# Jiawei-Yang/Denoising-ViT

Measured on AMD Instinct MI355X. Metric: stage-1 images denoised/sec (DINOv2-B/14, 518px, 1k Adam steps), higher is better.
Workload: dtype bf16

## Files before the change

denoising-vit_amd/csrc/dvt_fit_fused.hip:

```cpp
#include "dvt_common.h"
#include "dvt_grid_dev.h"
#include "dvt_loss_row.h"

typedef short bf16x8 __attribute__((ext_vector_type(8)));
typedef float f32x4 __attribute__((ext_vector_type(4)));

int g_fit_rows32 = 1;
int g_fit_xcd_affinity = 1;
int g_fit_small_wg = 0;

namespace {

constexpr int FR0 = 16;
constexpr int FW8 = 8;
constexpr int FE = 128;

template <bool F32>
struct Op {
  static constexpr int ES = F32 ? 4 : 2;
  static constexpr int KS = F32 ? 16 : 32;
};
typedef unsigned u32x4f __attribute__((ext_vector_type(4)));

template <bool F32>
__host__ __device__ constexpr int apitch(int K) { return K * Op<F32>::ES + 16; }

struct FusedArgs {
  DvtGridTable T;
  DvtShadowLayout S;
  DvtTLayout TL;
  int n, lattice;
  int xcd_group;
  float grad_scale;
  long long off_grid, off_b1, off_b2, off_G, off_bh1, off_bh2, off_bh3;
  DvtFusedFit f[DVT_FIT_BATCH_MAX];
};

__device__ __forceinline__ uint16_t bf16_of(float v) { return (uint16_t)(dvt_pack_bf16x2(v, 0.f) & 0xffffu); }

template <int NC, int FR, int FW, bool F32>
__device__ __forceinline__ void store_T(const char* img, void* __restrict__ dstTv, int B, int b0, int tid) {
  constexpr int RPP = F32 ? 4 : 8;
  for (int item = tid; item < NC * (FR / RPP); item += 64 * FW) {
    const int grp = item / NC, col = item - grp * NC;
    const int brow = b0 + grp * RPP;
    const char* src = img + grp * RPP * apitch<F32>(NC) + col * Op<F32>::ES;
    if constexpr (F32) {
      const int sg = brow >> 4, g = (brow >> 2) & 3;
      float4 v;
      v.x = *reinterpret_cast<const float*>(src);
      v.y = *reinterpret_cast<const float*>(src + apitch<F32>(NC));
      v.z = *reinterpret_cast<const float*>(src + 2 * apitch<F32>(NC));
      v.w = *reinterpret_cast<const float*>(src + 3 * apitch<F32>(NC));
      const long long off = ((long long)(col >> 4) * (B >> 4) + sg) * 256 + (((g << 4) + (col & 15)) << 2);
      *reinterpret_cast<float4*>(static_cast<float*>(dstTv) + off) = v;
    } else {
      const int kstep = brow >> 5, g = (brow >> 3) & 3;
      uint32_t w[4];
#pragma unroll
      for (int j = 0; j < 4; ++j) {
        const uint32_t lo = *reinterpret_cast<const uint16_t*>(src + (2 * j) * apitch<F32>(NC));
        const uint32_t hi = *reinterpret_cast<const uint16_t*>(src + (2 * j + 1) * apitch<F32>(NC));
        w[j] = lo | (hi << 16);
      }
      const long long off = ((long long)(col >> 4) * (B >> 5) + kstep) * 512 + (((g << 4) + (col & 15)) << 3);
      *reinterpret_cast<uint4*>(static_cast<uint16_t*>(dstTv) + off) = make_uint4(w[0], w[1], w[2], w[3]);
    }
  }
}

template <int K, int N, bool RELU, bool MASK, int RB, int FW, bool F32>
__device__ __forceinline__ void mlp_layer(const char* actA, const void* __restrict__ Wv,
                                          const float* __restrict__ bias, char* act_out,
                                          float* __restrict__ gout, const char* mask, int wave, int lane) {
  constexpr int KS = Op<F32>::KS, ES = Op<F32>::ES;
  constexpr int NTILES = N / 16, NT = (NTILES + FW - 1) / FW, S = K / KS;
  constexpr int INFL = FW == 8 ? 24 : 16;
  constexpr int PD0 = INFL / NT > 16 ? 16 : (INFL / NT < 1 ? 1 : INFL / NT);
  constexpr int PD = PD0 < S ? PD0 : S;
  static_assert(K % KS == 0 && N % 16 == 0, "layer shape");
  const int lc = lane & 15, g = lane >> 4;
  f32x4 acc[RB][NT];
  const char* wp[NT];
#pragma unroll
  for (int i = 0; i < NT; ++i) {
#pragma unroll
    for (int rb = 0; rb < RB; ++rb) acc[rb][i] = (f32x4){0.f, 0.f, 0.f, 0.f};
    const int t = wave + FW * i;
    const int tt = (NTILES % FW == 0 || t < NTILES) ? t : 0;
    wp[i] = static_cast<const char*>(Wv) + (size_t)tt * S * 1024 + lane * 16;
  }
  u32x4f b[PD][NT];
#pragma unroll
  for (int p = 0; p < PD; ++p)
#pragma unroll
    for (int i = 0; i < NT; ++i) b[p][i] = *reinterpret_cast<const u32x4f*>(wp[i] + 1024 * p);
  __builtin_amdgcn_sched_barrier(0);
  const char* ap = actA + lc * apitch<F32>(K) + g * 16;
#pragma unroll
  for (int s = 0; s < S; ++s) {
    u32x4f av[RB];
#pragma unroll
    for (int rb = 0; rb < RB; ++rb) av[rb] = *reinterpret_cast<const u32x4f*>(ap + rb * 16 * apitch<F32>(K) + s * 64);
    if constexpr (F32) {
#pragma unroll
      for (int j = 0; j < 4; ++j)
#pragma unroll
        for (int i = 0; i < NT; ++i)
#pragma unroll
          for (int rb = 0; rb < RB; ++rb)
            acc[rb][i] = __builtin_amdgcn_mfma_f32_16x16x4f32(__uint_as_float(av[rb][j]), __uint_as_float(b[s % PD][i][j]),
                                                              acc[rb][i], 0, 0, 0);
    } else {
#pragma unroll
      for (int i = 0; i < NT; ++i)
#pragma unroll
        for (int rb = 0; rb < RB; ++rb)
          acc[rb][i] = __builtin_amdgcn_mfma_f32_16x16x32_bf16(__builtin_bit_cast(bf16x8, av[rb]),
                                                               __builtin_bit_cast(bf16x8, b[s % PD][i]), acc[rb][i], 0, 0, 0);
    }
    if (s + PD < S) {
#pragma unroll
      for (int i = 0; i < NT; ++i) b[s % PD][i] = *reinterpret_cast<const u32x4f*>(wp[i] + 1024 * (s + PD));
    }
    __builtin_amdgcn_sched_barrier(0);
  }
#pragma unroll
  for (int i = 0; i < NT; ++i) {
    const int t = wave + FW * i;
    if (NTILES % FW != 0 && t >= NTILES) continue;
    const int n = t * 16 + lc;
    const float bv = bias != nullptr ? bias[n] : 0.f;
#pragma unroll
    for (int rb = 0; rb < RB; ++rb)
#pragma unroll
      for (int r = 0; r < 4; ++r) {
        const int row = rb * 16 + 4 * g + r;
        float v = acc[rb][i][r] + bv;
        if (RELU) v = fmaxf(v, 0.f);
        if (MASK) {
          if constexpr (F32) {
            v = *reinterpret_cast<const float*>(mask + row * apitch<F32>(N) + n * ES) > 0.f ? v : 0.f;
          } else {
            const uint16_t m = *reinterpret_cast<const uint16_t*>(mask + row * apitch<F32>(N) + n * ES);
            v = (m != 0 && !(m & 0x8000u)) ? v : 0.f;
          }
        }
        if (act_out != nullptr) {
          if constexpr (F32) *reinterpret_cast<float*>(act_out + row * apitch<F32>(N) + n * ES) = v;
          else *reinterpret_cast<uint16_t*>(act_out + row * apitch<F32>(N) + n * ES) = bf16_of(v);
        }
        if (gout != nullptr) gout[(size_t)row * N + n] = v;
      }
  }
}

template <int C, bool PH2, int FR, bool F32 = false>
struct FusedLds {
  static constexpr int H = C / 2, R = C / 4;
  static constexpr int O_ENC = 0;
  static constexpr int O_H1 = O_ENC + FR * apitch<F32>(FE);
  static constexpr int O_DF = O_H1 + FR * apitch<F32>(H);
  static constexpr int O_RAW = O_DF + FR * apitch<F32>(C);
  static constexpr int O_R1 = O_RAW + FR * apitch<F32>(C);
  static constexpr int O_R2 = O_R1 + FR * apitch<F32>(R);
  static constexpr int TOTAL = PH2 ? O_R2 + FR * apitch<F32>(R) : O_RAW;
};
template <int C>
constexpr bool fused_f32_fits() { return FusedLds<C, true, 16, true>::TOTAL <= 160 * 1024; }

template <int C, bool PH2, int FR, int FW, bool F32 = false>
__global__ __launch_bounds__(64 * FW) void fit_rows_kernel(FusedArgs a) {
  using L = FusedLds<C, PH2, FR, F32>;
  constexpr int RB = FR / 16;
  constexpr int ES = Op<F32>::ES;
  static_assert(FR == 16 || FR == 32, "rows per workgroup");
  static_assert(FW == 8 || (FW == 4 && FR == 16), "waves per workgroup");
  static_assert(!F32 || (FR == 16 && FW == 8), "fp32 operands: 16 rows, 8 waves");
  static_assert(L::TOTAL <= 160 * 1024, "LDS images of the row kernel");
  constexpr int H = C / 2, R = C / 4, E = FE, cq = C / 4;
  __shared__ __attribute__((aligned(16))) char smem[L::TOTAL];
  int fit_, rb_;
  if (a.xcd_group > 0) {
    const int lin = (int)blockIdx.x + (int)blockIdx.y * (int)gridDim.x, xcd = lin & 7, j = lin >> 3;
    fit_ = xcd / a.xcd_group;
    rb_ = j * a.xcd_group + xcd % a.xcd_group;
  } else {
    fit_ = (int)blockIdx.y;
    rb_ = (int)blockIdx.x;
  }
  const DvtFusedFit& f = a.f[fit_];
  const int tid = threadIdx.x, lane = tid & 63;
  const int wave = __builtin_amdgcn_readfirstlane(tid >> 6);
  const int row0 = rb_ * FR;
  const char* __restrict__ sh = static_cast<const char*>(f.shadow);
  const float* __restrict__ P = f.params;
  const float4* __restrict__ feat4 = reinterpret_cast<const float4*>(f.feat);

  uint32_t warm[5] = {0u, 0u, 0u, 0u, 0u};
  {
    constexpr int LPR = (C * 4 + 127) / 128;
    const int j = lane % 32;
#pragma unroll
    for (int rr = lane / 32; rr < FR / FW; rr += 2) {
      if (j < LPR) {
        const int ri = f.ridx[row0 + wave + FW * rr];
        warm[4] ^= __float_as_uint(f.feat[(size_t)ri * C + j * 32]) ^
                   __float_as_uint(P[a.off_G + (size_t)(ri % a.lattice) * C + j * 32]);
      }
    }
  }
  {
    const int per_xcd = a.xcd_group > 0 ? (int)gridDim.x / a.xcd_group : ((int)gridDim.x + 7) / 8;
    const int nslot = per_xcd >= 16 ? 16 : per_xcd;
    const int slot = (a.xcd_group > 0 ? rb_ / a.xcd_group : (rb_ >> 3)) % nslot;
    const long long lines = ((PH2 ? a.S.total : a.S.direct[2]) * ES + 127) / 128;
    const long long per = (lines + nslot - 1) / nslot;
    const long long l0 = slot * per, l1 = l0 + per < lines ? l0 + per : lines;
    const uint32_t* w32 = reinterpret_cast<const uint32_t*>(sh);
#pragma unroll
    for (int j = 0; j < 4 * RB * (8 / FW); ++j) {
      const long long li = l0 + tid + (long long)j * 64 * FW;
      if (li < l1) warm[j & 3] ^= w32[li * 32];
    }
  }

  if (tid < FR * 16) {
    const int r = tid >> 4, l = tid & 15;
    const float2 p = reinterpret_cast<const float2*>(f.xy)[f.ridx[row0 + r]];
    uint32_t idx[4];
    float w[4];
    corners2d(a.T, l, p.x, p.y, idx, w);
    const float4* __restrict__ grid = reinterpret_cast<const float4*>(P + a.off_grid);
    float4 lo = make_float4(0.f, 0.f, 0.f, 0.f), hi = lo;
#pragma unroll
    for (int c = 0; c < 4; ++c) {
      const float4 u = grid[(size_t)idx[c] * 2], v = grid[(size_t)idx[c] * 2 + 1];
      lo.x = fmaf(w[c], u.x, lo.x);
      lo.y = fmaf(w[c], u.y, lo.y);
      lo.z = fmaf(w[c], u.z, lo.z);
      lo.w = fmaf(w[c], u.w, lo.w);
      hi.x = fmaf(w[c], v.x, hi.x);
      hi.y = fmaf(w[c], v.y, hi.y);
      hi.z = fmaf(w[c], v.z, hi.z);
      hi.w = fmaf(w[c], v.w, hi.w);
    }
    if constexpr (F32) {
      *reinterpret_cast<float4*>(smem + L::O_ENC + r * apitch<F32>(E) + l * 32) = lo;
      *reinterpret_cast<float4*>(smem + L::O_ENC + r * apitch<F32>(E) + l * 32 + 16) = hi;
    } else {
      *reinterpret_cast<uint4*>(smem + L::O_ENC + r * apitch<F32>(E) + l * 16) =
          make_uint4(dvt_pack_bf16x2(lo.x, lo.y), dvt_pack_bf16x2(lo.z, lo.w), dvt_pack_bf16x2(hi.x, hi.y),
                     dvt_pack_bf16x2(hi.z, hi.w));
    }
  }
  if (PH2) {
    for (int i = tid; i < FR * cq; i += 64 * FW) {
      const int r = i / cq, q = i - r * cq;
      const float4 v = feat4[(size_t)f.ridx[row0 + r] * cq + q];
      if constexpr (F32)
        *reinterpret_cast<float4*>(smem + L::O_RAW + r * apitch<F32>(C) + q * 16) = v;
      else
        *reinterpret_cast<uint2*>(smem + L::O_RAW + r * apitch<F32>(C) + q * 8) =
            make_uint2(dvt_pack_bf16x2(v.x, v.y), dvt_pack_bf16x2(v.z, v.w));
    }
  }
  __syncthreads();

  const int B = a.n;
  char* __restrict__ T = static_cast<char*>(f.T);
#define SH(off) (sh + (size_t)(off) * ES)
#define TT(idx) (T + (size_t)a.TL.off[idx] * ES)
  mlp_layer<E, H, true, false, RB, FW, F32>(smem + L::O_ENC, SH(a.S.direct[0]), P + a.off_b1, smem + L::O_H1, nullptr,
                               nullptr, wave, lane);
  if (PH2)
    mlp_layer<C, R, true, false, RB, FW, F32>(smem + L::O_RAW, SH(a.S.direct[2]), P + a.off_bh1, smem + L::O_R1, nullptr,
                                 nullptr, wave, lane);
  __syncthreads();
  mlp_layer<H, C, false, false, RB, FW, F32>(smem + L::O_H1, SH(a.S.direct[1]), P + a.off_b2, nullptr,
                                f.F + (size_t)row0 * C, nullptr, wave, lane);
  store_T<H, FR, FW, F32>(smem + L::O_H1, TT(DVT_T_H1), B, row0, tid);
  store_T<E, FR, FW, F32>(smem + L::O_ENC, TT(DVT_T_ENC), B, row0, tid);
  if (PH2) {
    mlp_layer<R, R, true, false, RB, FW, F32>(smem + L::O_R1, SH(a.S.direct[3]), P + a.off_bh2, smem + L::O_R2, nullptr,
                                 nullptr, wave, lane);
    store_T<C, FR, FW, F32>(smem + L::O_RAW, TT(DVT_T_RAW), B, row0, tid);
    store_T<R, FR, FW, F32>(smem + L::O_R1, TT(DVT_T_R1), B, row0, tid);
    __syncthreads();
    mlp_layer<R, C, false, false, RB, FW, F32>(smem + L::O_R2, SH(a.S.direct[4]), P + a.off_bh3, nullptr,
                                  f.Hres + (size_t)row0 * C, nullptr, wave, lane);
    store_T<R, FR, FW, F32>(smem + L::O_R2, TT(DVT_T_R2), B, row0, tid);
  }
  __syncthreads();

  static_assert(C <= 1024, "row warm-up above assumes <= 32 lines per row");
  {
    constexpr int NR = FR / FW;
    constexpr int NB = (C <= 768 && !(FW == 4 && PH2)) ? 2 : 1;
    DvtLossRowRegs<PH2> lr[NB];
#pragma unroll
    for (int r0 = 0; r0 < NR; r0 += NB) {
#pragma unroll
    for (int rr = r0; rr < r0 + NB; ++rr) {
      const int gr = row0 + wave + FW * rr;
      const int ri = f.ridx[gr];
      dvt_loss_row_load<PH2>(lr[rr - r0], reinterpret_cast<const float4*>(f.F) + (size_t)gr * cq,
                             reinterpret_cast<const float4*>(P + a.off_G) + (size_t)(ri % a.lattice) * cq,
                             PH2 ? reinterpret_cast<const float4*>(f.Hres) + (size_t)gr * cq : nullptr,
                             feat4 + (size_t)ri * cq, cq, lane);
    }
#pragma unroll
// ... 140 lines not shown
                                                                  __builtin_bit_cast(bf16x8, fb[q][j]), acc[i][j], 0, 0, 0);
        }
        if (do_bias) {
#pragma unroll
          for (int i = 0; i < 2; ++i) {
            if constexpr (F32) {
#pragma unroll
              for (int e = 0; e < 4; ++e) bsum[i] += __uint_as_float(fa[q][i][e]);
            } else {
#pragma unroll
              for (int e = 0; e < 4; ++e) {
                bsum[i] += __uint_as_float(fa[q][i][e] << 16);
                bsum[i] += __uint_as_float(fa[q][i][e] & 0xffff0000u);
              }
            }
          }
        }
        if (s0 + q + PD < S) {
#pragma unroll
          for (int i = 0; i < 2; ++i) {
            fa[q][i] = *reinterpret_cast<const u32x4f*>(ap[i] + 1024 * (s0 + q + PD));
            fb[q][i] = *reinterpret_cast<const u32x4f*>(bp[i] + 1024 * (s0 + q + PD));
          }
        }
        __builtin_amdgcn_sched_barrier(0);
      }
    }
#pragma unroll
    for (int i = 0; i < 2; ++i)
#pragma unroll
      for (int j = 0; j < 2; ++j)
#pragma unroll
        for (int r = 0; r < 4; ++r) mine[((i * 2 + j) * 4 + r) * 64 + lane] = acc[i][j][r];
    if (do_bias) {
#pragma unroll
      for (int i = 0; i < 2; ++i) {
        float v = bsum[i];
        v += __shfl_xor(v, 16, 64);
        v += __shfl_xor(v, 32, 64);
        if (lane < 16) mine[1024 + i * 16 + lane] = v;
      }
    }
  }
  __syncthreads();
  if (is_w) {
    if (ks != 0) return;
    const float* base = red + slot * 4 * WG_PART_FLOATS;
    const int lc = lane & 15, g = lane >> 4;
#pragma unroll
    for (int i = 0; i < 2; ++i)
#pragma unroll
      for (int j = 0; j < 2; ++j)
#pragma unroll
        for (int r = 0; r < 4; ++r) {
          const int o = ((i * 2 + j) * 4 + r) * 64 + lane;
          const float v = (base[o] + base[WG_PART_FLOATS + o]) + (base[2 * WG_PART_FLOATS + o] + base[3 * WG_PART_FLOATS + o]);
          out_w[(size_t)(mb * 32 + i * 16 + 4 * g + r) * out_n + nb * 32 + j * 16 + lc] = v;
        }
    if (do_bias && lane < 32) {
      const int o = 1024 + lane;
      out_b[mb * 32 + lane] = (base[o] + base[WG_PART_FLOATS + o]) + (base[2 * WG_PART_FLOATS + o] + base[3 * WG_PART_FLOATS + o]);
    }
    return;
  }
  const int u = gu * 4 + ks;
  if (u >= a.n_gather * a.lattice) return;
  const int fi = u / a.lattice, r = u - fi * a.lattice;
  const WgradGather& gg = a.gg[fi];
  const int o0 = gg.offs[r], o1 = gg.offs[r + 1];
  if (o1 == o0) return;
  for (int q = lane; q < a.cq; q += 64) {
    float4 acc4 = make_float4(0.f, 0.f, 0.f, 0.f);
    for (int o = o0; o < o1; ++o) {
      const float4 d = gg.rows[(size_t)gg.perm[o] * a.cq + q];
      acc4.x += d.x;
      acc4.y += d.y;
      acc4.z += d.z;
      acc4.w += d.w;
    }
    gg.dG[(size_t)r * a.cq + q] = acc4;
  }
}

struct BackwardArgs {
  DvtGridTable T;
  GridBwdPlan plan;
  GridBwdPtrs gp;
  GridSortedPtrs gs;
  int n, grid_blocks_per_fit, k, wg_blocks;
  WgradArgs w;
};
template <int WAVES, bool F32 = false>
__global__ __launch_bounds__(64 * WAVES) void fit_backward_kernel(BackwardArgs a) {
  __shared__ __attribute__((aligned(16))) float smem[WAVES * WG_PART_FLOATS];
  if ((int)blockIdx.x >= a.wg_blocks) {
    const int b = (int)blockIdx.x - a.wg_blocks;
    const int fy = b / a.grid_blocks_per_fit, bx = b - fy * a.grid_blocks_per_fit;
    if (a.gs.nt > 0) {
      const int parts = a.gs.nt / (64 * WAVES);
      grid_gather_body(a.T, a.gs, fy, bx / parts, bx % parts, a.gp.d_enc[fy], a.gp.d_params[fy], a.gp.touched[fy], 64 * WAVES);
      return;
    }
    if constexpr (WAVES == 16)
      grid_bwd_body<256>(a.T, a.plan, a.gp, a.n, bx, fy, smem, reinterpret_cast<uint32_t*>(smem + 256 * 8));
    return;
  }
  const int wave = __builtin_amdgcn_readfirstlane(threadIdx.x >> 6);
  wgrad_block<WAVES / 4, F32>(a.w, (int)blockIdx.x, wave, threadIdx.x & 63, smem);
}

template <int C>
int launch_rows(const FusedArgs& a, int k, bool phase2, hipStream_t s) {
  if (a.S.f32) {
    if constexpr (fused_f32_fits<C>()) {
      dim3 grid(a.n / 16, k), block(64 * FW8);
      if (phase2) hipLaunchKernelGGL((fit_rows_kernel<C, true, 16, FW8, true>), grid, block, 0, s, a);
      else hipLaunchKernelGGL((fit_rows_kernel<C, false, 16, FW8, true>), grid, block, 0, s, a);
      DVT_CHECK_LAUNCH();
      return 0;
    }
    return DVT_E_BADARG;
  }
  const bool fits32 = phase2 ? (FusedLds<C, true, 32>::TOTAL <= 160 * 1024) : (FusedLds<C, false, 32>::TOTAL <= 160 * 1024);
  const bool r32 = fits32 && a.n % 32 == 0 && (g_fit_rows32 == 2 || (g_fit_rows32 == 1 && k >= 4));
  const bool small = g_fit_small_wg && !r32;
  dim3 grid(a.n / (r32 ? 32 : 16), k), block(64 * (small ? 4 : FW8));
  FusedArgs ax = a;
  ax.xcd_group = (g_fit_xcd_affinity && (k == 2 || k == 4) && grid.x % (8 / k) == 0 && (grid.x * k) % 8 == 0) ? 8 / k : 0;
  const FusedArgs& a_ = ax;
  if (r32) {
    if (phase2) {
      if constexpr (FusedLds<C, true, 32>::TOTAL <= 160 * 1024) hipLaunchKernelGGL((fit_rows_kernel<C, true, 32, FW8>), grid, block, 0, s, a_);
    } else {
      if constexpr (FusedLds<C, false, 32>::TOTAL <= 160 * 1024) hipLaunchKernelGGL((fit_rows_kernel<C, false, 32, FW8>), grid, block, 0, s, a_);
    }
  } else if (small) {
    if (phase2) hipLaunchKernelGGL((fit_rows_kernel<C, true, 16, 4>), grid, block, 0, s, a_);
    else hipLaunchKernelGGL((fit_rows_kernel<C, false, 16, 4>), grid, block, 0, s, a_);
  } else if (phase2) {
    hipLaunchKernelGGL((fit_rows_kernel<C, true, 16, FW8>), grid, block, 0, s, a_);
  } else {
    hipLaunchKernelGGL((fit_rows_kernel<C, false, 16, FW8>), grid, block, 0, s, a_);
  }
  DVT_CHECK_LAUNCH();
  return 0;
}

}

int dvt_shadow_layout(const DvtFitConfig* c, DvtShadowLayout* L) {
  if (!c || !L) return DVT_E_BADARG;
  const int C = c->feat_dim, H = c->hidden, R = c->res_hidden;
  const int E = c->grid.n_levels * c->grid.n_features;
  const int Ns[DVT_SHADOW_MATS] = {H, C, R, R, C}, Ks[DVT_SHADOW_MATS] = {E, H, C, R, R};
  const long long begins[DVT_SHADOW_MATS] = {c->off_w1, c->off_w2, c->off_wh1, c->off_wh2, c->off_wh3};
  const bool tr[DVT_SHADOW_MATS] = {true, true, false, true, true};
  long long o = 0;
  L->n = DVT_SHADOW_MATS;
  L->f32 = c->mlp_bf16 ? 0 : 1;
  L->lo = begins[0];
  L->hi = 0;
  for (int i = 0; i < DVT_SHADOW_MATS; ++i) {
    if (Ks[i] % 32 || Ns[i] % 16 || (tr[i] && (Ns[i] % 32 || Ks[i] % 16))) return DVT_E_BADARG;
    L->N[i] = Ns[i];
    L->K[i] = Ks[i];
    L->begin[i] = begins[i];
    const long long sz = (long long)Ns[i] * Ks[i];
    L->direct[i] = o;
    o += sz;
    L->transp[i] = tr[i] ? o : -1;
    if (tr[i]) o += sz;
    if (begins[i] < L->lo) L->lo = begins[i];
    if (begins[i] + sz > L->hi) L->hi = begins[i] + sz;
  }
  L->total = o;
  return 0;
}

int dvt_shadow_build_k(const DvtShadowLayout* L, int k, const float* const* params, void* const* shadow,
                       long long lo, long long hi, hipStream_t s) {
  if (!L || k < 1 || k > DVT_FIT_BATCH_MAX || L->n <= 0) return DVT_E_BADARG;
  const float* p[4] = {nullptr, nullptr, nullptr, nullptr};
  void* sh[4] = {nullptr, nullptr, nullptr, nullptr};
  for (int f = 0; f < k; ++f) {
    if (!params[f] || !shadow[f]) return DVT_E_BADARG;
    p[f] = params[f];
    sh[f] = shadow[f];
  }
  const long long q_lo = (lo > L->lo ? lo : L->lo) / 4, q_hi = (hi < L->hi ? hi : L->hi) / 4;
  if (q_hi <= q_lo) return 0;
  hipLaunchKernelGGL(shadow_build_kernel, dim3(dvt_cdiv(q_hi - q_lo, 256), k), dim3(256), 0, s, *L, p[0], p[1],
                     p[2], p[3], sh[0], sh[1], sh[2], sh[3], q_lo, q_hi);
  DVT_CHECK_LAUNCH();
  return 0;
}

int g_fit_fused_enable = 1;
int g_fit_sorted_grid = 1;

int g_fit_fused_f32 = 1;

bool dvt_fit_fused_ok(const DvtFitConfig* c) {
  if (!g_fit_fused_enable || !c || !dvt_fit_fused_shapes_ok(c)) return false;
  if (c->mlp_bf16) return true;
  return g_fit_fused_f32 && (c->feat_dim == 384 || c->feat_dim == 768);
}

bool dvt_fit_fused_shapes_ok(const DvtFitConfig* c) {
  if (!c) return false;
  if (c->grid.n_levels != 16 || c->grid.n_features != 8) return false;
  const int C = c->feat_dim;
  if (C != 384 && C != 768 && C != 1024) return false;
  if (c->hidden != C / 2 || c->res_hidden != C / 4) return false;
  if (c->batch % 512 || c->batch <= 0) return false;
  return c->lattice <= 8192 && c->batch <= 65535;
}

int dvt_fit_rows_k(const DvtFitConfig* c, const DvtShadowLayout* L, int k, const DvtFusedFit* fits, bool phase2,
                   hipStream_t s) {
  if (!dvt_fit_fused_ok(c) || !L || !fits || k < 1 || k > DVT_FIT_BATCH_MAX) return DVT_E_BADARG;
  FusedArgs a{};
  a.T = c->grid;
  a.S = *L;
  dvt_t_layout(c, &a.TL);
  a.n = c->batch;
  a.lattice = c->lattice;
  a.grad_scale = (float)c->grad_scale;
  a.off_grid = c->off_grid;
  a.off_b1 = c->off_b1;
  a.off_b2 = c->off_b2;
  a.off_G = c->off_G;
  a.off_bh1 = c->off_bh1;
  a.off_bh2 = c->off_bh2;
  a.off_bh3 = c->off_bh3;
  for (int f = 0; f < k; ++f) a.f[f] = fits[f];
  const double C = c->feat_dim, H = c->hidden, R = c->res_hidden, E = FE, B = c->batch;
  const double flops = 2.0 * B * (2.0 * (E * H + H * C) + (phase2 ? (C * R + 2.0 * R * R + 2.0 * R * C) : 0.0));
  DvtProbeScope probe(DVT_PROBE_FIT_ROWS, s, flops * k);
  switch (c->feat_dim) {
    case 384: return launch_rows<384>(a, k, phase2, s);
    case 768: return launch_rows<768>(a, k, phase2, s);
    default: return launch_rows<1024>(a, k, phase2, s);
  }
}

void dvt_t_layout(const DvtFitConfig* c, DvtTLayout* L) {
  const int C = c->feat_dim, H = c->hidden, R = c->res_hidden, E = c->grid.n_levels * c->grid.n_features;
  const int cols[DVT_T_COUNT] = {C, H, H, E, C, R, R, C, R, R};
  long long o = 0;
  for (int i = 0; i < DVT_T_COUNT; ++i) {
    L->off[i] = o;
    L->cols[i] = cols[i];
    o += (long long)cols[i] * c->batch;
  }
  L->total = o;
}

int dvt_fit_backward_k(const DvtFitConfig* c, int k, const DvtFusedFit* fits, bool phase2, hipStream_t s) {
  if (!dvt_fit_fused_ok(c) || !fits || k < 1 || k > DVT_FIT_BATCH_MAX) return DVT_E_BADARG;
  DvtTLayout TL;
  dvt_t_layout(c, &TL);
  const int C = c->feat_dim, H = c->hidden, R = c->res_hidden, E = c->grid.n_levels * c->grid.n_features;
  BackwardArgs ba{};
  WgradArgs& a = ba.w;
  a.B = c->batch;
  const int ksteps = a.B / 32;
  a.ksplit = 4;
  if (ksteps % 16) return DVT_E_BADARG;
  int units = 0;
  double flops = 0.0;
  const bool f32 = !c->mlp_bf16;
  const size_t es = f32 ? 4 : 2;
  auto add = [&](const DvtFusedFit& f, int tA, int tB, long long ow, long long ob, int M, int N) {
    WgradProb& p = a.p[a.n_prob];
    p.AT = static_cast<const char*>(f.T) + (size_t)TL.off[tA] * es;
    p.BT = static_cast<const char*>(f.T) + (size_t)TL.off[tB] * es;
    p.dW = f.grads + ow;
    p.db = f.grads + ob;
    p.M = M;
    p.N = N;
    a.unit0[a.n_prob++] = units;
    units += (M / 32) * (N / 32);
    flops += 2.0 * M * N * a.B;
  };
  for (int f = 0; f < k; ++f) {
    add(fits[f], DVT_T_DF, DVT_T_H1, c->off_w2, c->off_b2, C, H);
    add(fits[f], DVT_T_DH1, DVT_T_ENC, c->off_w1, c->off_b1, H, E);
    if (phase2) {
      add(fits[f], DVT_T_DH, DVT_T_R2, c->off_wh3, c->off_bh3, C, R);
      add(fits[f], DVT_T_DR2, DVT_T_R1, c->off_wh2, c->off_bh2, R, R);
      add(fits[f], DVT_T_DR1, DVT_T_RAW, c->off_wh1, c->off_bh1, R, C);
    }
  }
  a.unit0[a.n_prob] = units;
  a.units_total = units;
  a.lattice = c->lattice;
  a.cq = C / 4;
  if (!phase2) {
    for (int f = 0; f < k; ++f) {
      if (!fits[f].g_offs || !fits[f].g_perm) return DVT_E_BADARG;
      a.gg[f] = WgradGather{fits[f].g_offs, fits[f].g_perm, reinterpret_cast<const float4*>(fits[f].dF),
                            reinterpret_cast<float4*>(fits[f].grads + c->off_G)};
    }
    a.n_gather = k;
  }
  ba.T = c->grid;
  ba.n = c->batch;
  ba.k = k;
  const int saved_chunk = g_grid_lds_chunk;
  g_grid_lds_chunk = 256;
  dvt_grid_bwd_plan(c->grid, c->batch, &ba.plan);
  g_grid_lds_chunk = saved_chunk;
  const long long direct_threads = (long long)c->batch * (c->grid.n_levels - ba.plan.first_direct_level) * 8;
  ba.grid_blocks_per_fit = ba.plan.n_lds_blocks + dvt_cdiv(direct_threads, 1024);
  bool sorted = g_fit_sorted_grid && dvt_grid_sorted_ok(&c->grid, c->batch);
  for (int f = 0; f < k; ++f) sorted = sorted && fits[f].gs_keys && fits[f].gs_pay && fits[f].gs_w;
  const bool small = g_fit_small_wg && sorted && !f32;
  if (sorted) {
    ba.gs.nt = 4 * c->batch;
    ba.gs.bitmap_end = fits[0].gs_bitmap_end;
    ba.grid_blocks_per_fit = c->grid.n_levels * (ba.gs.nt / (small ? 512 : 1024));
    for (int f = 0; f < k; ++f) {
      ba.gs.keys[f] = fits[f].gs_keys;
      ba.gs.pay[f] = fits[f].gs_pay;
      ba.gs.w[f] = fits[f].gs_w;
    }
  }
  for (int f = 0; f < k; ++f) {
    ba.gp.xy[f] = reinterpret_cast<const float2*>(fits[f].xy);
    ba.gp.ridx[f] = fits[f].ridx;
    ba.gp.d_enc[f] = fits[f].denc;
    ba.gp.d_params[f] = fits[f].grads + c->off_grid;
    ba.gp.touched[f] = fits[f].touched;
  }
  const int wg_blocks = dvt_cdiv((long long)units + dvt_cdiv((long long)a.n_gather * a.lattice, 4), small ? 2 : 4);
  ba.wg_blocks = wg_blocks;
  DvtProbeScope probe(DVT_PROBE_FIT_GEMM, s, flops);
  if (f32)
    hipLaunchKernelGGL((fit_backward_kernel<16, true>), dim3(ba.grid_blocks_per_fit * k + wg_blocks), dim3(1024), 0, s, ba);
  else if (small)
    hipLaunchKernelGGL(fit_backward_kernel<8>, dim3(ba.grid_blocks_per_fit * k + wg_blocks), dim3(512), 0, s, ba);
  else
    hipLaunchKernelGGL(fit_backward_kernel<16>, dim3(ba.grid_blocks_per_fit * k + wg_blocks), dim3(1024), 0, s, ba);
  DVT_CHECK_LAUNCH();
  return 0;
}
```

denoising-vit_amd/csrc/dvt_gemm_f32.hip:

```cpp
#include "dvt_common.h"

typedef float floatx16 __attribute__((ext_vector_type(16)));

namespace {

constexpr int BK = 64;
constexpr int LDK = BK + 4;

struct GemmArgs {
  const float* A;
  const float* B;
  float* C;
  int M, N, K;
  int lda, ldb, ldc;
  const float* bias;
  const float* mask;
  int ldmask;
  float* colsum;
  int relu;
  int kchunk;
  int atomic;
  int epi;
  const float* gamma;
  const float* smul;
// ... 718 lines not shown
  const int tiles = dvt_cdiv(n, 64) * dvt_cdiv(k, 64);
  const int ktiles = dvt_cdiv(m, 64);
  int splits = dvt_cdiv(384, tiles);
  if (splits > ktiles / 2) splits = ktiles / 2;
  if (splits < 1) splits = 1;
  a.kchunk = dvt_cdiv(ktiles, splits) * 64;
  *splits_out = dvt_cdiv(m, a.kchunk);
  return a;
}

GemmArgs make_dgrad(const float* dy, const float* w, float* dx, const float* relu_mask, int m,
                    int n, int k) {
  GemmArgs a{};
  a.A = dy; a.B = w; a.C = dx;
  a.M = m; a.N = k; a.K = n;
  a.lda = n; a.ldb = k; a.ldc = k;
  a.mask = relu_mask; a.ldmask = k;
  a.kchunk = (n + 63) / 64 * 64;
  return a;
}

}

int dvt_linear_group(const DvtLinearOp* ops, int n_ops, hipStream_t s, int bf16_operands) {
  if (!ops || n_ops < 1 || n_ops > MULTI_MAX) return DVT_E_BADARG;
  MultiArgs m{};
  m.n = n_ops;
  int blocks = 0;
  double flops = 0.0;
  for (int i = 0; i < n_ops; ++i) {
    const DvtLinearOp& o = ops[i];
    if (o.m <= 0 || o.n <= 0 || o.k <= 0 || (o.n & 3) || (o.k & 3)) return DVT_E_BADARG;
    int splits = 1;
    if (o.kind == 0) {
      m.g[i] = make_fwd(o.x, o.w, o.b, o.y, o.m, o.n, o.k, o.relu);
      m.layout[i] = 0;
    } else if (o.kind == 1) {
      m.g[i] = make_wgrad(o.dy, o.x, o.dw, o.db, o.m, o.n, o.k, &splits);
      m.layout[i] = 2;
    } else if (o.kind == 2) {
      m.g[i] = make_dgrad(o.dy, o.w, o.dx, o.relu_mask, o.m, o.n, o.k);
      m.layout[i] = 1;
    } else {
      return DVT_E_BADARG;
    }
    m.gx[i] = dvt_cdiv(m.g[i].N, 64);
    m.gy[i] = dvt_cdiv(m.g[i].M, 64);
    m.blk0[i] = blocks;
    blocks += m.gx[i] * m.gy[i] * splits;
    flops += 2.0 * o.m * o.n * o.k;
  }
  m.blk0[n_ops] = blocks;
  DvtProbeScope probe(DVT_PROBE_FIT_GEMM, s, flops);
  if (bf16_operands) {
    if (g_f32_bk == 64)
      hipLaunchKernelGGL(gemm_bf16op_multi_kernel<64>, dim3(blocks), dim3(256), 0, s, m);
    else
      hipLaunchKernelGGL(gemm_bf16op_multi_kernel<32>, dim3(blocks), dim3(256), 0, s, m);
  } else if (g_f32_bk == 16)
    hipLaunchKernelGGL(gemm_f32_multi_kernel<16>, dim3(blocks), dim3(256), 0, s, m);
  else if (g_f32_bk == 32)
    hipLaunchKernelGGL(gemm_f32_multi_kernel<32>, dim3(blocks), dim3(256), 0, s, m);
  else
    hipLaunchKernelGGL(gemm_f32_multi_kernel<64>, dim3(blocks), dim3(256), 0, s, m);
  DVT_CHECK_LAUNCH();
  return 0;
}

namespace {
extern int g_cfg_override;
}
extern int g_fit_fused_enable;
extern int g_fit_fused_f32;
extern int g_fit_sorted_grid;
extern int g_fit_lazy_adam;
extern int g_fit_lazy_refresh;
extern int g_fit_lazy_exact;
extern int g_fit_lazy_merge;
extern int g_fit_shadow_in_adam;
extern int g_adam_pingpong;
extern int g_fit_rows32;
extern int g_fit_small_wg;
extern int g_fit_xcd_affinity;
#ifdef DVT_LAB
extern int g_fit_skip_mask;
#endif

extern "C" int dvt_tune_set(int key, int value) {
  if (key == 0) {
    g_cfg_override = value;
    return 0;
  }
  if (key == 4) {
    if (value == 2 || value == 3)
      g_f32_ex_stages = value;
    else if (value == 10 || value == 11)
      g_f32_big = value == 11;
    else
      g_f32_glds = value;
    return 0;
  }
  if (key == 5) {
    if (value != 16 && value != 32 && value != 64) return DVT_E_BADARG;
    g_f32_bk = value;
    return 0;
  }
  if (key == 8) {
    g_adam_pingpong = value != 0;
    return 0;
  }
  if (key == 6) {
    if (value == 2 || value == 3)
      g_fit_fused_f32 = value == 3;
    else
      g_fit_fused_enable = value != 0;
    return 0;
  }
  if (key == 7) {
    g_fit_sorted_grid = value != 0;
    return 0;
  }
  if (key == 10) {
    g_fit_lazy_exact = value != 0;
    return 0;
  }
  if (key == 11) {
    g_fit_lazy_merge = value != 0;
    return 0;
  }
  if (key == 12) {
    g_fit_shadow_in_adam = value != 0;
    return 0;
  }
  if (key == 13) {
    if (value < 0 || value > 2) return DVT_E_BADARG;
    g_fit_rows32 = value;
    return 0;
  }
  if (key == 14) {
    g_fit_small_wg = value != 0;
    return 0;
  }
  if (key == 16) {
    g_fit_xcd_affinity = value != 0;
    return 0;
  }
#ifdef DVT_LAB
  if (key == 15) {
    g_fit_skip_mask = value & 7;
    return 0;
  }
#endif
  if (key == 9) {
    g_fit_lazy_adam = value != 0;
    if (value >= 2) g_fit_lazy_refresh = value;
    return 0;
  }
  if (key == 18) return dvt_s2_tune(value);
  if (key == 1) return dvt_vit_tune(value);
  if (key == 2) return dvt_grid_tune(value);
  if (key == 3) return dvt_adam_tune(value);
  return DVT_E_BADARG;
}

int dvt_gemm_f32_ex(const DvtGemmEx* g, hipStream_t s) {
  if (!g || !g->A || !g->B || !g->C || g->M <= 0 || g->N <= 0 || g->K <= 0) return DVT_E_BADARG;
  GemmArgs a{};
  a.A = g->A; a.B = g->B; a.C = g->C;
  a.M = g->M; a.N = g->N; a.K = g->K;
  a.lda = g->lda; a.ldb = g->ldb; a.ldc = g->ldc;
  a.bias = g->bias;
  a.colsum = g->layout == 2 ? g->colsum : nullptr;
  a.atomic = g->accumulate;
  if (g->smul != nullptr) {
    const int nb_ = (g->nb0 > 0 ? g->nb0 : 1) * (g->nb1 > 0 ? g->nb1 : 1);
    if (!g->rowsub || g->layout != 0 || nb_ <= 1 || g->K > BK || g->accumulate) return DVT_E_BADARG;
    a.smul = g->smul;
    a.rowsub = g->rowsub;
    a.oscale = g->oscale;
  }
  if (a.K % BK) return DVT_E_BADARG;
  const bool a_kc = g->layout != 2, b_kc = g->layout == 0;
  if ((!a_kc && (a.M % 64)) || (!b_kc && (a.N % 64)) || (a.lda & 3) || (a.ldb & 3)) return DVT_E_BADARG;
  const int nb = (g->nb0 > 0 ? g->nb0 : 1) * (g->nb1 > 0 ? g->nb1 : 1);
  int splits = 1;
  a.kchunk = a.K;
  if (g->accumulate && nb == 1) {
    const int tiles = dvt_cdiv(a.M, 64) * dvt_cdiv(a.N, 64), ktiles = a.K / BK;
    splits = dvt_cdiv(1024, tiles);
    if (splits > ktiles / 4) splits = ktiles / 4;
    if (splits < 1) splits = 1;
    a.kchunk = dvt_cdiv(ktiles, splits) * BK;
    splits = dvt_cdiv(a.K, a.kchunk);
  }
  if (nb > 65535 || splits > 65535) return DVT_E_BADARG;
  dim3 grid(dvt_cdiv(a.N, 64), dvt_cdiv(a.M, 64), nb > 1 ? nb : splits);
  DvtProbeScope probe(DVT_PROBE_FIT_GEMM, s, 2.0 * a.M * a.N * a.K * nb);
#define EX_LAUNCH(NS)                                                                                     \
  do {                                                                                                    \
    if (nb > 1) {                                                                                         \
      BatchDims d{g->nb1 > 0 ? g->nb1 : 1, g->sA0, g->sA1, g->sB0, g->sB1, g->sC0, g->sC1};               \
      if (a.K <= BK && g->layout == 0)                                                                    \
        hipLaunchKernelGGL((gemm_f32_batched_small_k_kernel<true, true>), grid, dim3(256), 0, s, a, d);   \
      else if (g->layout == 0)                                                                            \
        hipLaunchKernelGGL((gemm_f32_glds_batched_kernel<true, true, NS>), grid, dim3(256), 0, s, a, d);  \
      else if (g->layout == 1)                                                                            \
        hipLaunchKernelGGL((gemm_f32_glds_batched_kernel<true, false, NS>), grid, dim3(256), 0, s, a, d); \
      else                                                                                                \
        hipLaunchKernelGGL((gemm_f32_glds_batched_kernel<false, false, NS>), grid, dim3(256), 0, s, a, d);\
    } else {                                                                                              \
      if (g->layout == 0)                                                                                 \
        hipLaunchKernelGGL((gemm_f32_glds_kernel<true, true, NS>), grid, dim3(256), 0, s, a);             \
      else if (g->layout == 1)                                                                            \
        hipLaunchKernelGGL((gemm_f32_glds_kernel<true, false, NS>), grid, dim3(256), 0, s, a);            \
      else                                                                                                \
        hipLaunchKernelGGL((gemm_f32_glds_kernel<false, false, NS>), grid, dim3(256), 0, s, a);           \
    }                                                                                                     \
  } while (0)
  if (g_f32_ex_stages == 2)
    EX_LAUNCH(2);
  else
    EX_LAUNCH(3);
#undef EX_LAUNCH
  DVT_CHECK_LAUNCH();
  return 0;
}

// ... 92 lines not shown
```

Measured before the change: 3.011.

## Add 64-row fused fit tiles and 32x64 weight-gradient units

Adds a 64-rows-per-workgroup variant of the fused row kernel. To fit in LDS it aliases the encoding image inside the d(pred) buffer, and it is enabled by default when k>=4. It also adds a wider weight-gradient block in which each unit computes a 32x64 tile with 2x4 MFMA accumulators and double-buffered register prefetch. This halves the unit count and increases operand reuse per load. Both raise register and LDS pressure and may lower occupancy or parallelism for small problem sizes.

```diff
diff --git a/denoising-vit_amd/csrc/dvt_fit_fused.hip b/denoising-vit_amd/csrc/dvt_fit_fused.hip
--- a/denoising-vit_amd/csrc/dvt_fit_fused.hip
+++ b/denoising-vit_amd/csrc/dvt_fit_fused.hip
@@ -7,6 +7,7 @@
 
 int g_fit_rows32 = 1;
 int g_fit_xcd_affinity = 1;
+int g_fit_wgrad_wide = 1;
 int g_fit_small_wg = 0;
 
 namespace {
@@ -158,10 +159,11 @@
 template <int C, bool PH2, int FR, bool F32 = false>
 struct FusedLds {
   static constexpr int H = C / 2, R = C / 4;
+  static constexpr bool AL = FR == 64;
   static constexpr int O_ENC = 0;
-  static constexpr int O_H1 = O_ENC + FR * apitch<F32>(FE);
-  static constexpr int O_DF = O_H1 + FR * apitch<F32>(H);
-  static constexpr int O_RAW = O_DF + FR * apitch<F32>(C);
+  static constexpr int O_H1 = AL ? FR * apitch<F32>(C) : FR * apitch<F32>(FE);
+  static constexpr int O_DF = AL ? 0 : O_H1 + FR * apitch<F32>(H);
+  static constexpr int O_RAW = O_H1 + FR * apitch<F32>(H) + (AL ? 0 : FR * apitch<F32>(C));
   static constexpr int O_R1 = O_RAW + FR * apitch<F32>(C);
   static constexpr int O_R2 = O_R1 + FR * apitch<F32>(R);
   static constexpr int TOTAL = PH2 ? O_R2 + FR * apitch<F32>(R) : O_RAW;
@@ -174,8 +176,9 @@
   using L = FusedLds<C, PH2, FR, F32>;
   constexpr int RB = FR / 16;
   constexpr int ES = Op<F32>::ES;
-  static_assert(FR == 16 || FR == 32, "rows per workgroup");
+  static_assert(FR == 16 || FR == 32 || FR == 64, "rows per workgroup");
   static_assert(FW == 8 || (FW == 4 && FR == 16), "waves per workgroup");
+  static_assert(!L::AL || L::O_ENC + FR * apitch<F32>(FE) <= L::O_DF + FR * apitch<F32>(C), "enc inside the d(pred) image");
   static_assert(!F32 || (FR == 16 && FW == 8), "fp32 operands: 16 rows, 8 waves");
   static_assert(L::TOTAL <= 160 * 1024, "LDS images of the row kernel");
   constexpr int H = C / 2, R = C / 4, E = FE, cq = C / 4;
@@ -225,8 +228,8 @@
     }
   }
 
-  if (tid < FR * 16) {
-    const int r = tid >> 4, l = tid & 15;
+  for (int it = tid; it < FR * 16; it += 64 * FW) {
+    const int r = it >> 4, l = it & 15;
     const float2 p = reinterpret_cast<const float2*>(f.xy)[f.ridx[row0 + r]];
     uint32_t idx[4];
     float w[4];
@@ -533,6 +536,142 @@
   }
 }
 
+template <int SLOTS>
+__device__ __forceinline__ void wgrad_block_wide(const WgradArgs& a, int blk, int wave, int lane, float* red) {
+  constexpr int PD = 2;
+  const int slot = wave >> 2, ks = wave & 3;
+  const int unit = blk * SLOTS + slot;
+  float* mine = red + (slot * 4 + ks) * WG_PART_FLOATS;
+  const bool is_w = unit < a.units_total;
+  const int gu = unit - a.units_total;
+  float* out_w = nullptr;
+  float* out_b = nullptr;
+  int out_n = 0;
+  int mb = 0, nb = 0;
+  bool do_bias = false;
+  f32x4 acc[2][4];
+  float bsum[2] = {0.f, 0.f};
+  if (is_w) {
+    int pi = 0;
+#pragma unroll
+    for (int j = 1; j < WG_MAX_PROB; ++j)
+      if (j < a.n_prob && unit >= a.unit0[j]) pi = j;
+    const WgradProb& p = a.p[pi];
+    out_w = p.dW;
+    out_b = p.db;
+    out_n = p.N;
+    const int local = unit - a.unit0[pi], nbn = p.N >> 6;
+    mb = local / nbn;
+    nb = local - mb * nbn;
+    const int ksteps = a.B / 32, S = ksteps >> 2, s_begin = ks * S;
+    const char* ap[2];
+    const char* bp[4];
+#pragma unroll
+    for (int i = 0; i < 2; ++i) ap[i] = p.AT + ((size_t)(mb * 2 + i) * ksteps + s_begin) * 1024 + lane * 16;
+#pragma unroll
+    for (int j = 0; j < 4; ++j) bp[j] = p.BT + ((size_t)(nb * 4 + j) * ksteps + s_begin) * 1024 + lane * 16;
+#pragma unroll
+    for (int i = 0; i < 2; ++i)
+#pragma unroll
+      for (int j = 0; j < 4; ++j) acc[i][j] = (f32x4){0.f, 0.f, 0.f, 0.f};
+    do_bias = p.db != nullptr && nb == 0;
+    u32x4f fa[PD][2], fb[PD][4];
+#pragma unroll
+    for (int q = 0; q < PD; ++q) {
+#pragma unroll
+      for (int i = 0; i < 2; ++i) fa[q][i] = *reinterpret_cast<const u32x4f*>(ap[i] + 1024 * q);
+#pragma unroll
+      for (int j = 0; j < 4; ++j) fb[q][j] = *reinterpret_cast<const u32x4f*>(bp[j] + 1024 * q);
+    }
+    __builtin_amdgcn_sched_barrier(0);
+    for (int s0 = 0; s0 < S; s0 += PD) {
+#pragma unroll
+      for (int q = 0; q < PD; ++q) {
+#pragma unroll
+        for (int i = 0; i < 2; ++i)
+#pragma unroll
+          for (int j = 0; j < 4; ++j)
+            acc[i][j] = __builtin_amdgcn_mfma_f32_16x16x32_bf16(__builtin_bit_cast(bf16x8, fa[q][i]),
+                                                                __builtin_bit_cast(bf16x8, fb[q][j]), acc[i][j], 0, 0, 0);
+        if (do_bias) {
+#pragma unroll
+          for (int i = 0; i < 2; ++i)
+#pragma unroll
+            for (int e = 0; e < 4; ++e) {
+              bsum[i] += __uint_as_float(fa[q][i][e] << 16);
+              bsum[i] += __uint_as_float(fa[q][i][e] & 0xffff0000u);
+            }
+        }
+        if (s0 + q + PD < S) {
+#pragma unroll
+          for (int i = 0; i < 2; ++i) fa[q][i] = *reinterpret_cast<const u32x4f*>(ap[i] + 1024 * (s0 + q + PD));
+#pragma unroll
+          for (int j = 0; j < 4; ++j) fb[q][j] = *reinterpret_cast<const u32x4f*>(bp[j] + 1024 * (s0 + q + PD));
+        }
+        __builtin_amdgcn_sched_barrier(0);
+      }
+    }
+  }
+  const int lc = lane & 15, g = lane >> 4;
+#pragma unroll
+  for (int h = 0; h < 2; ++h) {
+    if (is_w) {
+#pragma unroll
+      for (int i = 0; i < 2; ++i)
+#pragma unroll
+        for (int jj = 0; jj < 2; ++jj)
+#pragma unroll
+          for (int r = 0; r < 4; ++r) mine[((i * 2 + jj) * 4 + r) * 64 + lane] = acc[i][2 * h + jj][r];
+      if (h == 0 && do_bias) {
+#pragma unroll
+        for (int i = 0; i < 2; ++i) {
+          float v = bsum[i];
+          v += __shfl_xor(v, 16, 64);
+          v += __shfl_xor(v, 32, 64);
+          if (lane < 16) mine[1024 + i * 16 + lane] = v;
+        }
+      }
+    }
+    __syncthreads();
+    if (is_w && ks == 0) {
+      const float* base = red + slot * 4 * WG_PART_FLOATS;
+#pragma unroll
+      for (int i = 0; i < 2; ++i)
+#pragma unroll
+        for (int jj = 0; jj < 2; ++jj)
+#pragma unroll
+          for (int r = 0; r < 4; ++r) {
+            const int o = ((i * 2 + jj) * 4 + r) * 64 + lane;
+            const float v = (base[o] + base[WG_PART_FLOATS + o]) + (base[2 * WG_PART_FLOATS + o] + base[3 * WG_PART_FLOATS + o]);
+            out_w[(size_t)(mb * 32 + i * 16 + 4 * g + r) * out_n + nb * 64 + (2 * h + jj) * 16 + lc] = v;
+          }
+      if (h == 0 && do_bias && lane < 32) {
+        const int o = 1024 + lane;
+        out_b[mb * 32 + lane] = (base[o] + base[WG_PART_FLOATS + o]) + (base[2 * WG_PART_FLOATS + o] + base[3 * WG_PART_FLOATS + o]);
+      }
+    }
+    if (h == 0) __syncthreads();
+  }
+  if (is_w) return;
+  const int u = gu * 4 + ks;
+  if (u >= a.n_gather * a.lattice) return;
+  const int fi = u / a.lattice, r = u - fi * a.lattice;
+  const WgradGather& gg = a.gg[fi];
+  const int o0 = gg.offs[r], o1 = gg.offs[r + 1];
+  if (o1 == o0) return;
+  for (int q = lane; q < a.cq; q += 64) {
+    float4 acc4 = make_float4(0.f, 0.f, 0.f, 0.f);
+    for (int o = o0; o < o1; ++o) {
+      const float4 d = gg.rows[(size_t)gg.perm[o] * a.cq + q];
+      acc4.x += d.x;
+      acc4.y += d.y;
+      acc4.z += d.z;
+      acc4.w += d.w;
+    }
+    gg.dG[(size_t)r * a.cq + q] = acc4;
+  }
+}
+
 struct BackwardArgs {
   DvtGridTable T;
   GridBwdPlan plan;
@@ -541,8 +680,9 @@
   int n, grid_blocks_per_fit, k, wg_blocks;
   WgradArgs w;
 };
-template <int WAVES, bool F32 = false>
+template <int WAVES, bool F32 = false, bool WIDE = false>
 __global__ __launch_bounds__(64 * WAVES) void fit_backward_kernel(BackwardArgs a) {
+  static_assert(!(F32 && WIDE), "32 x 64 weight-gradient units: bf16 operands");
   __shared__ __attribute__((aligned(16))) float smem[WAVES * WG_PART_FLOATS];
   if ((int)blockIdx.x >= a.wg_blocks) {
     const int b = (int)blockIdx.x - a.wg_blocks;
@@ -557,9 +697,11 @@
     return;
   }
   const int wave = __builtin_amdgcn_readfirstlane(threadIdx.x >> 6);
-  wgrad_block<WAVES / 4, F32>(a.w, (int)blockIdx.x, wave, threadIdx.x & 63, smem);
-}
-
+  if constexpr (WIDE) wgrad_block_wide<WAVES / 4>(a.w, (int)blockIdx.x, wave, threadIdx.x & 63, smem);
+  else wgrad_block<WAVES / 4, F32>(a.w, (int)blockIdx.x, wave, threadIdx.x & 63, smem);
+}
+
+constexpr bool FIT_ROWS64_AUTO = true;
 template <int C>
 int launch_rows(const FusedArgs& a, int k, bool phase2, hipStream_t s) {
   if (a.S.f32) {
@@ -572,14 +714,23 @@
     }
     return DVT_E_BADARG;
   }
+  constexpr bool fits64_p1 = FusedLds<C, false, 64>::TOTAL <= 160 * 1024, fits64_p2 = FusedLds<C, true, 64>::TOTAL <= 160 * 1024;
+  const bool fits64 = phase2 ? fits64_p2 : fits64_p1;
+  const bool r64 = fits64 && a.n % 64 == 0 && (g_fit_rows32 == 3 || (g_fit_rows32 == 1 && k >= 4 && FIT_ROWS64_AUTO));
   const bool fits32 = phase2 ? (FusedLds<C, true, 32>::TOTAL <= 160 * 1024) : (FusedLds<C, false, 32>::TOTAL <= 160 * 1024);
-  const bool r32 = fits32 && a.n % 32 == 0 && (g_fit_rows32 == 2 || (g_fit_rows32 == 1 && k >= 4));
-  const bool small = g_fit_small_wg && !r32;
-  dim3 grid(a.n / (r32 ? 32 : 16), k), block(64 * (small ? 4 : FW8));
+  const bool r32 = !r64 && fits32 && a.n % 32 == 0 && (g_fit_rows32 >= 2 || (g_fit_rows32 == 1 && k >= 4));
+  const bool small = g_fit_small_wg && !r32 && !r64;
+  dim3 grid(a.n / (r64 ? 64 : (r32 ? 32 : 16)), k), block(64 * (small ? 4 : FW8));
   FusedArgs ax = a;
   ax.xcd_group = (g_fit_xcd_affinity && (k == 2 || k == 4) && grid.x % (8 / k) == 0 && (grid.x * k) % 8 == 0) ? 8 / k : 0;
   const FusedArgs& a_ = ax;
-  if (r32) {
+  if (r64) {
+    if (phase2) {
+      if constexpr (fits64_p2) hipLaunchKernelGGL((fit_rows_kernel<C, true, 64, FW8>), grid, block, 0, s, a_);
+    } else {
+      if constexpr (fits64_p1) hipLaunchKernelGGL((fit_rows_kernel<C, false, 64, FW8>), grid, block, 0, s, a_);
+    }
+  } else if (r32) {
     if (phase2) {
       if constexpr (FusedLds<C, true, 32>::TOTAL <= 160 * 1024) hipLaunchKernelGGL((fit_rows_kernel<C, true, 32, FW8>), grid, block, 0, s, a_);
     } else {
@@ -721,6 +872,8 @@
   int units = 0;
   double flops = 0.0;
   const bool f32 = !c->mlp_bf16;
+  const bool wide = g_fit_wgrad_wide && !f32 && H % 64 == 0 && E % 64 == 0 && (!phase2 || (R % 64 == 0 && C % 64 == 0));
+  const int unit_n = wide ? 64 : 32;
   const size_t es = f32 ? 4 : 2;
   auto add = [&](const DvtFusedFit& f, int tA, int tB, long long ow, long long ob, int M, int N) {
     WgradProb& p = a.p[a.n_prob];
@@ -731,7 +884,7 @@
     p.M = M;
     p.N = N;
     a.unit0[a.n_prob++] = units;
-    units += (M / 32) * (N / 32);
+    units += (M / 32) * (N / unit_n);
     flops += 2.0 * M * N * a.B;
   };
   for (int f = 0; f < k; ++f) {
@@ -787,12 +940,17 @@
   const int wg_blocks = dvt_cdiv((long long)units + dvt_cdiv((long long)a.n_gather * a.lattice, 4), small ? 2 : 4);
   ba.wg_blocks = wg_blocks;
   DvtProbeScope probe(DVT_PROBE_FIT_GEMM, s, flops);
+  const dim3 grid(ba.grid_blocks_per_fit * k + wg_blocks);
   if (f32)
-    hipLaunchKernelGGL((fit_backward_kernel<16, true>), dim3(ba.grid_blocks_per_fit * k + wg_blocks), dim3(1024), 0, s, ba);
+    hipLaunchKernelGGL((fit_backward_kernel<16, true>), grid, dim3(1024), 0, s, ba);
+  else if (small && wide)
+    hipLaunchKernelGGL((fit_backward_kernel<8, false, true>), grid, dim3(512), 0, s, ba);
   else if (small)
-    hipLaunchKernelGGL(fit_backward_kernel<8>, dim3(ba.grid_blocks_per_fit * k + wg_blocks), dim3(512), 0, s, ba);
+    hipLaunchKernelGGL(fit_backward_kernel<8>, grid, dim3(512), 0, s, ba);
+  else if (wide)
+    hipLaunchKernelGGL((fit_backward_kernel<16, false, true>), grid, dim3(1024), 0, s, ba);
   else
-    hipLaunchKernelGGL(fit_backward_kernel<16>, dim3(ba.grid_blocks_per_fit * k + wg_blocks), dim3(1024), 0, s, ba);
+    hipLaunchKernelGGL(fit_backward_kernel<16>, grid, dim3(1024), 0, s, ba);
   DVT_CHECK_LAUNCH();
   return 0;
 }
diff --git a/denoising-vit_amd/csrc/dvt_gemm_f32.hip b/denoising-vit_amd/csrc/dvt_gemm_f32.hip
--- a/denoising-vit_amd/csrc/dvt_gemm_f32.hip
+++ b/denoising-vit_amd/csrc/dvt_gemm_f32.hip
@@ -824,6 +824,7 @@
 extern int g_fit_rows32;
 extern int g_fit_small_wg;
 extern int g_fit_xcd_affinity;
+extern int g_fit_wgrad_wide;
 #ifdef DVT_LAB
 extern int g_fit_skip_mask;
 #endif
@@ -875,7 +876,7 @@
     return 0;
   }
   if (key == 13) {
-    if (value < 0 || value > 2) return DVT_E_BADARG;
+    if (value < 0 || value > 3) return DVT_E_BADARG;
     g_fit_rows32 = value;
     return 0;
   }
@@ -885,6 +886,10 @@
   }
   if (key == 16) {
     g_fit_xcd_affinity = value != 0;
+    return 0;
+  }
+  if (key == 17) {
+    g_fit_wgrad_wide = value != 0;
     return 0;
   }
 #ifdef DVT_LAB
```

After: 3.022 (median of 5 runs). No clear change (+0.4%).
